# OmicsML/dance

Measured on NVIDIA H100. Metric: cells/sec fwd+bwd scGNN, higher is better.
Workload: dtype f32 (wgmma 3xTF32 split GEMMs, fp32 everything else)

## Files before the change

dance_b200/csrc/gemm_tc.cu:

```cuda
#include "tc_common.cuh"

#include <cuda_bf16.h>
#include <stdlib.h>
#include <string.h>

namespace b2 {
namespace tc {

constexpr int BM = 128;
constexpr int BK = 32;
constexpr int CONSUMERS = 256;
constexpr int REWRITERS = 128;
constexpr int THREADS = CONSUMERS + REWRITERS;
constexpr int REWRITE_REGS = 80, CONSUMER_REGS = 208;
constexpr int MAX_STAGES = 4;
constexpr int SMEM_LIMIT = 227 * 1024;

enum Mode { MODE_TF32 = 0, MODE_TF32X3 = 1, MODE_BF16 = 2 };
__host__ __device__ constexpr int plane_row_bytes(int mode) { return mode == MODE_BF16 ? BK * 2 : BK * 4; }

struct Params {
  CUtensorMap tmA;
  CUtensorMap tmB;
  float* C;
  const float* bias;
  const float* mask;
  float* partial;
  long long ldc, ldmask;
  int M, N, K;
  int a_mn, b_mn;
  int mode;
  int act;
  float beta;
  int tiles_m, tiles_n, splits, kb_per_split, kb_total, stages, planes;
};

struct SmemLayout {
  uint32_t a_plane, b_plane, plane_buf, raw_a, raw_stage, ring, bars, total;
};
__host__ __device__ inline SmemLayout smem_layout(int BN, int mode, int stages, int planes) {
  SmemLayout L;
  L.a_plane = BM * plane_row_bytes(mode);
  L.b_plane = (uint32_t)BN * plane_row_bytes(mode);
  L.plane_buf = (mode == MODE_TF32X3 ? 2u : 1u) * (L.a_plane + L.b_plane);
  L.raw_a = BM * BK * 4;
  L.raw_stage = L.raw_a + (uint32_t)BN * BK * 4;
  L.ring = (uint32_t)planes * L.plane_buf;
  L.bars = L.ring + (uint32_t)stages * L.raw_stage;
  L.total = L.bars + 8 * 4 * MAX_STAGES;
  return L;
}

template <int MODE, int ROWS, bool MN>
__device__ __forceinline__ void convert_tile(const uint8_t* raw, uint8_t* hi, uint8_t* lo, int lt) {
  constexpr int PER = ROWS * (BK / 4) / REWRITERS;
  float4 v[PER];
#pragma unroll
  for (int j = 0; j < PER; ++j) {
    const int c = lt + j * REWRITERS;
    if constexpr (!MN) {
      v[j] = *reinterpret_cast<const float4*>(raw + (c >> 3) * 128 + (c & 7) * 16);
    } else {
      const float* col = reinterpret_cast<const float*>(raw) + c % ROWS + (c / ROWS) * 4 * ROWS;
      v[j] = make_float4(col[0], col[ROWS], col[2 * ROWS], col[3 * ROWS]);
    }
  }
#pragma unroll
  for (int j = 0; j < PER; ++j) {
    const int c = lt + j * REWRITERS;
    const uint32_t r = MN ? c % ROWS : c >> 3, kc = MN ? c / ROWS : c & 7;
    if constexpr (MODE == MODE_BF16) {
      const __nv_bfloat162 p0 = __floats2bfloat162_rn(v[j].x, v[j].y), p1 = __floats2bfloat162_rn(v[j].z, v[j].w);
      *reinterpret_cast<uint2*>(hi + sw64_offset16(r, kc * 4)) =
          make_uint2(*reinterpret_cast<const uint32_t*>(&p0), *reinterpret_cast<const uint32_t*>(&p1));
      continue;
    }
    const uint32_t off = sw128_offset32(r, kc * 4);
    if constexpr (MODE == MODE_TF32X3) {
      const float4 x = v[j];
      const float4 h = make_float4(__uint_as_float(__float_as_uint(x.x) & 0xFFFFE000u), __uint_as_float(__float_as_uint(x.y) & 0xFFFFE000u),
                                   __uint_as_float(__float_as_uint(x.z) & 0xFFFFE000u), __uint_as_float(__float_as_uint(x.w) & 0xFFFFE000u));
      *reinterpret_cast<float4*>(hi + off) = h;
      *reinterpret_cast<float4*>(lo + off) = make_float4(x.x - h.x, x.y - h.y, x.z - h.z, x.w - h.w);
    } else {
      *reinterpret_cast<float4*>(hi + off) = v[j];
    }
  }
}

template <int BN>
__device__ __forceinline__ void mma_ss(float (&d)[BN / 2], uint64_t a, uint64_t b, uint32_t scale_d) {
  if constexpr (BN == 32) wgmma_tf32_ss_n32(d, a, b, scale_d);
  else if constexpr (BN == 64) wgmma_tf32_ss_n64(d, a, b, scale_d);
  else wgmma_tf32_ss_n128(d, a, b, scale_d);
}
template <int BN>
__device__ __forceinline__ void mma_bf16_ss(float (&d)[BN / 2], uint64_t a, uint64_t b, uint32_t scale_d) {
  if constexpr (BN == 32) wgmma_bf16_ss_n32(d, a, b, scale_d);
  else if constexpr (BN == 64) wgmma_bf16_ss_n64(d, a, b, scale_d);
  else wgmma_bf16_ss_n128(d, a, b, scale_d);
}

template <int BN, int MODE>
__global__ void __launch_bounds__(THREADS, 1)
gemm_tc_kernel(const __grid_constant__ Params p) {
  extern __shared__ __align__(1024) uint8_t smem_raw[];
  uint8_t* smem = smem_raw + ((1024u - (smem_u32(smem_raw) & 1023u)) & 1023u);
  const SmemLayout L = smem_layout(BN, MODE, p.stages, p.planes);
  const uint32_t raw_full = smem_u32(smem + L.bars), raw_empty = raw_full + 8 * MAX_STAGES;
  const uint32_t plane_full = raw_empty + 8 * MAX_STAGES, plane_empty = plane_full + 8 * MAX_STAGES;
  const int tid = threadIdx.x, wg = tid >> 7, lt = tid & 127;

  const int u = blockIdx.x;
  const int ks = u % p.splits;
  const int t = u / p.splits;
  const int tn = t % p.tiles_n, tm = t / p.tiles_n;
  const int kb0 = ks * p.kb_per_split;
  const int nk = min(p.kb_total, kb0 + p.kb_per_split) - kb0;
  auto plane_ptrs = [&](int b, uint8_t*& a_hi, uint8_t*& a_lo, uint8_t*& b_hi, uint8_t*& b_lo) {
    a_hi = smem + b * L.plane_buf;
    a_lo = a_hi + L.a_plane;
    b_hi = a_hi + (MODE == MODE_TF32X3 ? 2 : 1) * L.a_plane;
    b_lo = b_hi + L.b_plane;
  };

  if (tid == 0) {
    tma_prefetch_desc(&p.tmA);
    tma_prefetch_desc(&p.tmB);
    for (int s = 0; s < p.stages; ++s) {
      mbar_init(raw_full + 8 * s, 1);
      mbar_init(raw_empty + 8 * s, REWRITERS);
    }
    for (int b = 0; b < p.planes; ++b) {
      mbar_init(plane_full + 8 * b, REWRITERS);
      mbar_init(plane_empty + 8 * b, CONSUMERS / 32);
    }
    fence_barrier_init();
  }
  __syncthreads();

  if (wg == 2) {
    asm volatile("setmaxnreg.dec.sync.aligned.u32 %0;" ::"n"(REWRITE_REGS));
    auto issue = [&](int i) {
      const int s = i % p.stages, kb = kb0 + i;
      const uint32_t fb = raw_full + 8 * s;
      const uint32_t ra = smem_u32(smem + L.ring + s * L.raw_stage), rb = ra + L.raw_a;
      mbar_expect_tx(fb, L.raw_stage);
      if (!p.a_mn) tma_load_2d(ra, &p.tmA, fb, kb * BK, tm * BM);
      else tma_load_2d(ra, &p.tmA, fb, tm * BM, kb * BK);
      if (!p.b_mn) tma_load_2d(rb, &p.tmB, fb, kb * BK, tn * BN);
      else tma_load_2d(rb, &p.tmB, fb, tn * BN, kb * BK);
    };
    if (lt == 0)
      for (int i = 0; i < min(nk, p.stages); ++i) issue(i);
    for (int i = 0; i < nk; ++i) {
      if (lt == 0 && i >= 1 && i - 1 + p.stages < nk) {
        mbar_wait(raw_empty + 8 * ((i - 1) % p.stages), (uint32_t)(((i - 1) / p.stages) & 1));
        issue(i - 1 + p.stages);
      }
      const int s = i % p.stages, b = i % p.planes;
      if (i >= p.planes) mbar_wait(plane_empty + 8 * b, (uint32_t)(((i / p.planes) - 1) & 1));
      mbar_wait(raw_full + 8 * s, (uint32_t)((i / p.stages) & 1));
      uint8_t *a_hi, *a_lo, *b_hi, *b_lo;
      plane_ptrs(b, a_hi, a_lo, b_hi, b_lo);
      const uint8_t* raw = smem + L.ring + s * L.raw_stage;
      if (p.a_mn) convert_tile<MODE, BM, true>(raw, a_hi, a_lo, lt);
      else convert_tile<MODE, BM, false>(raw, a_hi, a_lo, lt);
      if (p.b_mn) convert_tile<MODE, BN, true>(raw + L.raw_a, b_hi, b_lo, lt);
      else convert_tile<MODE, BN, false>(raw + L.raw_a, b_hi, b_lo, lt);
      mbar_arrive(raw_empty + 8 * s);
      fence_proxy_async();
      mbar_arrive(plane_full + 8 * b);
    }
    return;
  }

  asm volatile("setmaxnreg.inc.sync.aligned.u32 %0;" ::"n"(CONSUMER_REGS));
  float acc[BN / 2], acc_s[BN / 2];
  const int lane = lt & 31;
  for (int i = 0; i < nk; ++i) {
    const int b = i % p.planes;
    uint8_t *a_hi, *a_lo, *b_hi, *b_lo;
    plane_ptrs(b, a_hi, a_lo, b_hi, b_lo);
    mbar_wait(plane_full + 8 * b, (uint32_t)((i / p.planes) & 1));
    wgmma_fence();
    const uint32_t ah = smem_u32(a_hi) + wg * 64 * plane_row_bytes(MODE), al = smem_u32(a_lo) + wg * 64 * plane_row_bytes(MODE);
    const uint32_t bh = smem_u32(b_hi), bl = smem_u32(b_lo);
    if constexpr (MODE == MODE_BF16) {
#pragma unroll
      for (int k = 0; k < BK / 16; ++k) {
        const uint32_t ko = k * 16 * 2;
        mma_bf16_ss<BN>(acc, wgmma_desc_sw64(ah + ko), wgmma_desc_sw64(bh + ko), (i | k) != 0);
      }
    } else {
#pragma unroll
      for (int k = 0; k < BK / 8; ++k) {
        const uint32_t ko = k * 8 * 4;
        if constexpr (MODE == MODE_TF32X3) {
          mma_ss<BN>(acc_s, wgmma_desc_sw128(al + ko), wgmma_desc_sw128(bh + ko), (i | k) != 0);
          mma_ss<BN>(acc_s, wgmma_desc_sw128(ah + ko), wgmma_desc_sw128(bl + ko), 1);
        }
        mma_ss<BN>(acc, wgmma_desc_sw128(ah + ko), wgmma_desc_sw128(bh + ko), (i | k) != 0);
      }
    }
    wgmma_commit();
    wgmma_wait<1>();
    if (i >= 1 && lane == 0) mbar_arrive(plane_empty + 8 * ((i - 1) % p.planes));
  }
  wgmma_wait<0>();
  reg_fence(acc);
  if constexpr (MODE == MODE_TF32X3) reg_fence(acc_s);

  const int warp = lt >> 5;
  const int row_base = tm * BM + wg * 64 + warp * 16 + (lane >> 2);
  const bool vec_ok = ((p.ldc & 1) == 0) && ((reinterpret_cast<uintptr_t>(p.C) & 7) == 0);
#pragma unroll
  for (int v = 0; v < BN / 2; v += 2) {
    const int row = row_base + 8 * ((v >> 1) & 1);
    const int col = tn * BN + 8 * (v >> 2) + 2 * (lane & 3);
    if (row >= p.M || col >= p.N) continue;
    float o[2] = {acc[v], acc[v + 1]};
    if constexpr (MODE == MODE_TF32X3) { o[0] += acc_s[v]; o[1] += acc_s[v + 1]; }
    const bool two = col + 1 < p.N;
    if (p.partial) {
      float* dst = p.partial + ((size_t)ks * p.M + row) * p.N + col;
      dst[0] = o[0];
      if (two) dst[1] = o[1];
      continue;
    }
    float* dst = p.C + (size_t)row * p.ldc + col;
    const float* mrow = p.mask ? p.mask + (size_t)row * p.ldmask + col : nullptr;
#pragma unroll
    for (int jj = 0; jj < 2; ++jj) {
      if (jj == 1 && !two) break;
      float x = o[jj];
      if (p.bias) x += __ldg(p.bias + col + jj);
      x = apply_act(x, p.act);
      if (mrow && !(__ldg(mrow + jj) > 0.f)) x = 0.f;
      if (p.beta != 0.f) x = fmaf(p.beta, dst[jj], x);
      o[jj] = x;
    }
    if (two && vec_ok) *reinterpret_cast<float2*>(dst) = make_float2(o[0], o[1]);
    else { dst[0] = o[0]; if (two) dst[1] = o[1]; }
  }
}

__global__ void __launch_bounds__(256)
splitk_reduce_kernel(const float* __restrict__ partial, int splits, int M, int N, float* __restrict__ C, long long ldc,
                     const float* __restrict__ bias, int act, const float* __restrict__ mask, long long ldmask,
                     float beta) {
  const size_t total = (size_t)M * N;
  for (size_t i = (size_t)blockIdx.x * blockDim.x + threadIdx.x; i < total; i += (size_t)gridDim.x * blockDim.x) {
    const int r = (int)(i / N), c = (int)(i % N);
    float s = 0.f;
    for (int k = 0; k < splits; ++k) s += partial[(size_t)k * total + i];
    if (bias) s += bias[c];
    s = apply_act(s, act);
    if (mask && !(mask[(size_t)r * ldmask + c] > 0.f)) s = 0.f;
    float* dst = C + (size_t)r * ldc + c;
    if (beta != 0.f) s = fmaf(beta, *dst, s);
    *dst = s;
  }
}

typedef CUresult (*EncodeTiledFn)(CUtensorMap*, CUtensorMapDataType, cuuint32_t, void*, const cuuint64_t*,
                                  const cuuint64_t*, const cuuint32_t*, const cuuint32_t*, CUtensorMapInterleave,
                                  CUtensorMapSwizzle, CUtensorMapL2promotion, CUtensorMapFloatOOBfill);

static EncodeTiledFn get_encode() {
  static EncodeTiledFn fn = nullptr;
  static bool tried = false;
// ... 59 lines not shown
    splits = ceil_div(sms, tiles);
    const int max_splits = pl.kb_total / 4;
    if (splits > max_splits) splits = max_splits;
    if (splits < 1) splits = 1;
  }
  pl.kb_per_split = ceil_div(pl.kb_total, splits);
  pl.splits = ceil_div(pl.kb_total, pl.kb_per_split);
  return pl;
}

template <int BN, int MODE>
static int launch_gemm(const Params& p, const Plan& pl, cudaStream_t st) {
  static bool attr_set = false;
  if (!attr_set) {
    B2_CHECK_CUDA(cudaFuncSetAttribute(gemm_tc_kernel<BN, MODE>, cudaFuncAttributeMaxDynamicSharedMemorySize, SMEM_LIMIT));
    attr_set = true;
  }
  gemm_tc_kernel<BN, MODE><<<pl.tiles_m * pl.tiles_n * pl.splits, THREADS, pl.smem, st>>>(p);
  B2_CHECK_LAUNCH("gemm_tc_kernel");
  return B2_OK;
}

template <int MODE>
static int launch_gemm_mode(const Params& p, const Plan& pl, cudaStream_t st) {
  return pl.BN == 32 ? launch_gemm<32, MODE>(p, pl, st) : (pl.BN == 64 ? launch_gemm<64, MODE>(p, pl, st) : launch_gemm<128, MODE>(p, pl, st));
}

static int mode_of(int precision) {
  return precision == B2_PREC_TF32X3 ? MODE_TF32X3 : (precision == B2_PREC_BF16 ? MODE_BF16 : MODE_TF32);
}

}

size_t gemm_tc_workspace_bytes(int M, int N, int K, int transA, int transB, int precision) {
  if (M <= 0 || N <= 0 || K <= 0) return 0;
  const tc::Plan pl = tc::make_plan(M, N, K, tc::mode_of(precision));
  return pl.splits > 1 ? (size_t)pl.splits * M * N * sizeof(float) : 0;
}

int gemm_tc(const float* A, int64_t lda, int transA, const float* B, int64_t ldb, int transB, float* C, int64_t ldc,
            int M, int N, int K, const float* bias, int act, const float* mask, int64_t ldmask, float beta,
            int precision, void* workspace, size_t workspace_bytes, cudaStream_t st) {
  using namespace tc;
  if (K < 8 || (int64_t)M * N * K < (1ll << 18)) return B2_ERR_UNSUPPORTED;
  if ((reinterpret_cast<uintptr_t>(A) & 15) || (reinterpret_cast<uintptr_t>(B) & 15) || (lda & 3) || (ldb & 3))
    return B2_ERR_UNSUPPORTED;
  if (!get_encode()) return B2_ERR_UNSUPPORTED;

  const int mode = mode_of(precision);
  const Plan pl = make_plan(M, N, K, mode);
  Params p;
  memset(&p, 0, sizeof(p));
  const int NONE = (int)CU_TENSOR_MAP_SWIZZLE_NONE;
  const bool okA = transA ? make_tensor_map_f32_ex(&p.tmA, A, (uint64_t)M, (uint64_t)K, (uint64_t)lda, BM, BK, NONE)
                          : make_tensor_map_f32_ex(&p.tmA, A, (uint64_t)K, (uint64_t)M, (uint64_t)lda, BK, BM, NONE);
  const bool okB = transB ? make_tensor_map_f32_ex(&p.tmB, B, (uint64_t)K, (uint64_t)N, (uint64_t)ldb, BK, (uint32_t)pl.BN, NONE)
                          : make_tensor_map_f32_ex(&p.tmB, B, (uint64_t)N, (uint64_t)K, (uint64_t)ldb, (uint32_t)pl.BN, BK, NONE);
  if (!okA || !okB) return B2_ERR_UNSUPPORTED;
  p.C = C; p.bias = bias; p.mask = mask; p.ldc = ldc; p.ldmask = ldmask;
  p.M = M; p.N = N; p.K = K;
  p.a_mn = transA ? 1 : 0;
  p.b_mn = transB ? 0 : 1;
  p.mode = mode; p.act = act; p.beta = beta;
  p.tiles_m = pl.tiles_m; p.tiles_n = pl.tiles_n; p.splits = pl.splits; p.kb_per_split = pl.kb_per_split;
  p.kb_total = pl.kb_total; p.stages = pl.stages; p.planes = pl.planes;
  p.partial = nullptr;
  if (pl.splits > 1) {
    const size_t need = (size_t)pl.splits * M * N * sizeof(float);
    if (!workspace || workspace_bytes < need) {
      set_error("b2_gemm_f32: split-K workspace too small (%zu < %zu)", workspace_bytes, need);
      return B2_ERR_WORKSPACE;
    }
    p.partial = reinterpret_cast<float*>(workspace);
  }
  const int rc = mode == MODE_TF32X3 ? launch_gemm_mode<MODE_TF32X3>(p, pl, st)
               : (mode == MODE_BF16 ? launch_gemm_mode<MODE_BF16>(p, pl, st) : launch_gemm_mode<MODE_TF32>(p, pl, st));
  if (rc != B2_OK) return rc;
  if (pl.splits > 1) {
    size_t total = (size_t)M * N;
    int blocks = (int)((total + 255) / 256);
    if (blocks > sm_count() * 8) blocks = sm_count() * 8;
    splitk_reduce_kernel<<<blocks, 256, 0, st>>>(p.partial, pl.splits, M, N, C, ldc, bias, act, mask, ldmask, beta);
    B2_CHECK_LAUNCH("splitk_reduce_kernel");
  }
  return B2_OK;
}

}
```

dance_b200/csrc/tc_common.cuh:

```cuda
#pragma once
#include "common.cuh"

#include <cuda.h>

namespace b2 {
namespace tc {

__device__ __forceinline__ uint32_t smem_u32(const void* p) { return (uint32_t)__cvta_generic_to_shared(p); }

__device__ __forceinline__ void mbar_init(uint32_t bar, uint32_t count) {
  asm volatile("mbarrier.init.shared::cta.b64 [%0], %1;" ::"r"(bar), "r"(count));
}
__device__ __forceinline__ void mbar_expect_tx(uint32_t bar, uint32_t bytes) {
  asm volatile("mbarrier.arrive.expect_tx.shared::cta.b64 _, [%0], %1;" ::"r"(bar), "r"(bytes) : "memory");
}
__device__ __forceinline__ void mbar_arrive(uint32_t bar) {
  asm volatile("mbarrier.arrive.shared::cta.b64 _, [%0];" ::"r"(bar) : "memory");
}
__device__ __forceinline__ void mbar_wait(uint32_t bar, uint32_t parity) {
  asm volatile(
      "{\n\t"
      ".reg .pred p;\n\t"
      "WAIT_LOOP:\n\t"
      "mbarrier.try_wait.parity.shared::cta.b64 p, [%0], %1, %2;\n\t"
// ... 8 lines not shown
               : "=r"(ok) : "r"(bar), "r"(parity) : "memory");
  return ok != 0;
}
__device__ __forceinline__ void fence_barrier_init() { asm volatile("fence.mbarrier_init.release.cluster;" ::: "memory"); }
__device__ __forceinline__ void fence_proxy_async() { asm volatile("fence.proxy.async.shared::cta;" ::: "memory"); }
__device__ __forceinline__ void tma_load_2d(uint32_t dst, const CUtensorMap* map, uint32_t bar, int c0, int c1) {
  asm volatile(
      "cp.async.bulk.tensor.2d.shared::cluster.global.mbarrier::complete_tx::bytes [%0], [%1, {%3, %4}], [%2];"
      ::"r"(dst), "l"(map), "r"(bar), "r"(c0), "r"(c1) : "memory");
}
__device__ __forceinline__ void tma_prefetch_desc(const CUtensorMap* map) {
  asm volatile("prefetch.tensormap [%0];" ::"l"(map) : "memory");
}

__device__ __forceinline__ void bulk_load(uint32_t dst, const void* src, uint32_t bytes, uint32_t bar) {
  asm volatile("cp.async.bulk.shared::cluster.global.mbarrier::complete_tx::bytes [%0], [%1], %2, [%3];"
               ::"r"(dst), "l"(src), "r"(bytes), "r"(bar) : "memory");
}

__device__ __forceinline__ uint64_t wgmma_desc_sw128(uint32_t saddr) {
  uint64_t d = 0;
  d |= (uint64_t)((saddr & 0x3FFFF) >> 4);
  d |= (uint64_t)1 << 16;
  d |= (uint64_t)(1024 >> 4) << 32;
  d |= (uint64_t)1 << 62;
  return d;
}
__host__ __device__ __forceinline__ uint32_t sw128_offset32(uint32_t row, uint32_t k) {
  return row * 128u + ((((k >> 2) ^ row) & 7u) << 4) + (k & 3u) * 4u;
}
__device__ __forceinline__ uint64_t wgmma_desc_sw64(uint32_t saddr) {
  uint64_t d = 0;
  d |= (uint64_t)((saddr & 0x3FFFF) >> 4);
  d |= (uint64_t)1 << 16;
  d |= (uint64_t)(512 >> 4) << 32;
  d |= (uint64_t)2 << 62;
  return d;
}
__host__ __device__ __forceinline__ uint32_t sw64_offset16(uint32_t row, uint32_t k) {
  return row * 64u + ((((k >> 3) ^ (row >> 1)) & 3u) << 4) + (k & 7u) * 2u;
}
__host__ __device__ __forceinline__ uint32_t sw128_offset16(uint32_t row, uint32_t k) {
  return row * 128u + ((((k >> 3) ^ row) & 7u) << 4) + (k & 7u) * 2u;
}
__device__ __forceinline__ void wgmma_fence() { asm volatile("wgmma.fence.sync.aligned;" ::: "memory"); }
__device__ __forceinline__ void wgmma_commit() { asm volatile("wgmma.commit_group.sync.aligned;" ::: "memory"); }
template <int N>
__device__ __forceinline__ void wgmma_wait() { asm volatile("wgmma.wait_group.sync.aligned %0;" ::"n"(N) : "memory"); }
template <int R>
__device__ __forceinline__ void reg_fence(float (&d)[R]) {
#pragma unroll
  for (int i = 0; i < R; ++i) asm volatile("" : "+f"(d[i])::"memory");
}

__device__ __forceinline__ void wgmma_tf32_ss_n32(float (&d)[16], uint64_t a, uint64_t b, uint32_t scale_d) {
  asm volatile(
      "{\n\t.reg .pred p;\n\tsetp.ne.b32 p, %18, 0;\n\t"
      "wgmma.mma_async.sync.aligned.m64n32k8.f32.tf32.tf32 {%0, %1, %2, %3, %4, %5, %6, %7, %8, %9, %10, %11, %12, %13, %14, %15}, %16, %17, p, 1, 1;\n\t}\n"
      : "+f"(d[0]), "+f"(d[1]), "+f"(d[2]), "+f"(d[3]), "+f"(d[4]), "+f"(d[5]), "+f"(d[6]), "+f"(d[7]), "+f"(d[8]), "+f"(d[9]), "+f"(d[10]), "+f"(d[11]), "+f"(d[12]), "+f"(d[13]), "+f"(d[14]), "+f"(d[15])
      : "l"(a), "l"(b), "r"(scale_d));
}
__device__ __forceinline__ void wgmma_tf32_ss_n64(float (&d)[32], uint64_t a, uint64_t b, uint32_t scale_d) {
  asm volatile(
      "{\n\t.reg .pred p;\n\tsetp.ne.b32 p, %34, 0;\n\t"
      "wgmma.mma_async.sync.aligned.m64n64k8.f32.tf32.tf32 {%0, %1, %2, %3, %4, %5, %6, %7, %8, %9, %10, %11, %12, %13, %14, %15, %16, %17, %18, %19, %20, %21, %22, %23, %24, %25, %26, %27, %28, %29, %30, %31}, %32, %33, p, 1, 1;\n\t}\n"
      : "+f"(d[0]), "+f"(d[1]), "+f"(d[2]), "+f"(d[3]), "+f"(d[4]), "+f"(d[5]), "+f"(d[6]), "+f"(d[7]), "+f"(d[8]), "+f"(d[9]), "+f"(d[10]), "+f"(d[11]), "+f"(d[12]), "+f"(d[13]), "+f"(d[14]), "+f"(d[15]), "+f"(d[16]), "+f"(d[17]), "+f"(d[18]), "+f"(d[19]), "+f"(d[20]), "+f"(d[21]), "+f"(d[22]), "+f"(d[23]), "+f"(d[24]), "+f"(d[25]), "+f"(d[26]), "+f"(d[27]), "+f"(d[28]), "+f"(d[29]), "+f"(d[30]), "+f"(d[31])
      : "l"(a), "l"(b), "r"(scale_d));
}
__device__ __forceinline__ void wgmma_tf32_ss_n128(float (&d)[64], uint64_t a, uint64_t b, uint32_t scale_d) {
  asm volatile(
      "{\n\t.reg .pred p;\n\tsetp.ne.b32 p, %66, 0;\n\t"
      "wgmma.mma_async.sync.aligned.m64n128k8.f32.tf32.tf32 {%0, %1, %2, %3, %4, %5, %6, %7, %8, %9, %10, %11, %12, %13, %14, %15, %16, %17, %18, %19, %20, %21, %22, %23, %24, %25, %26, %27, %28, %29, %30, %31, %32, %33, %34, %35, %36, %37, %38, %39, %40, %41, %42, %43, %44, %45, %46, %47, %48, %49, %50, %51, %52, %53, %54, %55, %56, %57, %58, %59, %60, %61, %62, %63}, %64, %65, p, 1, 1;\n\t}\n"
      : "+f"(d[0]), "+f"(d[1]), "+f"(d[2]), "+f"(d[3]), "+f"(d[4]), "+f"(d[5]), "+f"(d[6]), "+f"(d[7]), "+f"(d[8]), "+f"(d[9]), "+f"(d[10]), "+f"(d[11]), "+f"(d[12]), "+f"(d[13]), "+f"(d[14]), "+f"(d[15]), "+f"(d[16]), "+f"(d[17]), "+f"(d[18]), "+f"(d[19]), "+f"(d[20]), "+f"(d[21]), "+f"(d[22]), "+f"(d[23]), "+f"(d[24]), "+f"(d[25]), "+f"(d[26]), "+f"(d[27]), "+f"(d[28]), "+f"(d[29]), "+f"(d[30]), "+f"(d[31]), "+f"(d[32]), "+f"(d[33]), "+f"(d[34]), "+f"(d[35]), "+f"(d[36]), "+f"(d[37]), "+f"(d[38]), "+f"(d[39]), "+f"(d[40]), "+f"(d[41]), "+f"(d[42]), "+f"(d[43]), "+f"(d[44]), "+f"(d[45]), "+f"(d[46]), "+f"(d[47]), "+f"(d[48]), "+f"(d[49]), "+f"(d[50]), "+f"(d[51]), "+f"(d[52]), "+f"(d[53]), "+f"(d[54]), "+f"(d[55]), "+f"(d[56]), "+f"(d[57]), "+f"(d[58]), "+f"(d[59]), "+f"(d[60]), "+f"(d[61]), "+f"(d[62]), "+f"(d[63])
      : "l"(a), "l"(b), "r"(scale_d));
}
__device__ __forceinline__ void wgmma_f16_ss_n64(float (&d)[32], uint64_t a, uint64_t b, uint32_t scale_d) {
  asm volatile(
      "{\n\t.reg .pred p;\n\tsetp.ne.b32 p, %34, 0;\n\t"
      "wgmma.mma_async.sync.aligned.m64n64k16.f32.f16.f16 {%0, %1, %2, %3, %4, %5, %6, %7, %8, %9, %10, %11, %12, %13, %14, %15, %16, %17, %18, %19, %20, %21, %22, %23, %24, %25, %26, %27, %28, %29, %30, %31}, %32, %33, p, 1, 1, 0, 0;\n\t}\n"
      : "+f"(d[0]), "+f"(d[1]), "+f"(d[2]), "+f"(d[3]), "+f"(d[4]), "+f"(d[5]), "+f"(d[6]), "+f"(d[7]), "+f"(d[8]), "+f"(d[9]), "+f"(d[10]), "+f"(d[11]), "+f"(d[12]), "+f"(d[13]), "+f"(d[14]), "+f"(d[15]), "+f"(d[16]), "+f"(d[17]), "+f"(d[18]), "+f"(d[19]), "+f"(d[20]), "+f"(d[21]), "+f"(d[22]), "+f"(d[23]), "+f"(d[24]), "+f"(d[25]), "+f"(d[26]), "+f"(d[27]), "+f"(d[28]), "+f"(d[29]), "+f"(d[30]), "+f"(d[31])
      : "l"(a), "l"(b), "r"(scale_d));
}
__device__ __forceinline__ void wgmma_bf16_ss_n32(float (&d)[16], uint64_t a, uint64_t b, uint32_t scale_d) {
  asm volatile(
      "{\n\t.reg .pred p;\n\tsetp.ne.b32 p, %18, 0;\n\t"
      "wgmma.mma_async.sync.aligned.m64n32k16.f32.bf16.bf16 {%0, %1, %2, %3, %4, %5, %6, %7, %8, %9, %10, %11, %12, %13, %14, %15}, %16, %17, p, 1, 1, 0, 0;\n\t}\n"
      : "+f"(d[0]), "+f"(d[1]), "+f"(d[2]), "+f"(d[3]), "+f"(d[4]), "+f"(d[5]), "+f"(d[6]), "+f"(d[7]), "+f"(d[8]), "+f"(d[9]), "+f"(d[10]), "+f"(d[11]), "+f"(d[12]), "+f"(d[13]), "+f"(d[14]), "+f"(d[15])
      : "l"(a), "l"(b), "r"(scale_d));
}
__device__ __forceinline__ void wgmma_bf16_ss_n64(float (&d)[32], uint64_t a, uint64_t b, uint32_t scale_d) {
  asm volatile(
      "{\n\t.reg .pred p;\n\tsetp.ne.b32 p, %34, 0;\n\t"
      "wgmma.mma_async.sync.aligned.m64n64k16.f32.bf16.bf16 {%0, %1, %2, %3, %4, %5, %6, %7, %8, %9, %10, %11, %12, %13, %14, %15, %16, %17, %18, %19, %20, %21, %22, %23, %24, %25, %26, %27, %28, %29, %30, %31}, %32, %33, p, 1, 1, 0, 0;\n\t}\n"
      : "+f"(d[0]), "+f"(d[1]), "+f"(d[2]), "+f"(d[3]), "+f"(d[4]), "+f"(d[5]), "+f"(d[6]), "+f"(d[7]), "+f"(d[8]), "+f"(d[9]), "+f"(d[10]), "+f"(d[11]), "+f"(d[12]), "+f"(d[13]), "+f"(d[14]), "+f"(d[15]), "+f"(d[16]), "+f"(d[17]), "+f"(d[18]), "+f"(d[19]), "+f"(d[20]), "+f"(d[21]), "+f"(d[22]), "+f"(d[23]), "+f"(d[24]), "+f"(d[25]), "+f"(d[26]), "+f"(d[27]), "+f"(d[28]), "+f"(d[29]), "+f"(d[30]), "+f"(d[31])
      : "l"(a), "l"(b), "r"(scale_d));
}
__device__ __forceinline__ void wgmma_bf16_ss_n128(float (&d)[64], uint64_t a, uint64_t b, uint32_t scale_d) {
  asm volatile(
      "{\n\t.reg .pred p;\n\tsetp.ne.b32 p, %66, 0;\n\t"
      "wgmma.mma_async.sync.aligned.m64n128k16.f32.bf16.bf16 {%0, %1, %2, %3, %4, %5, %6, %7, %8, %9, %10, %11, %12, %13, %14, %15, %16, %17, %18, %19, %20, %21, %22, %23, %24, %25, %26, %27, %28, %29, %30, %31, %32, %33, %34, %35, %36, %37, %38, %39, %40, %41, %42, %43, %44, %45, %46, %47, %48, %49, %50, %51, %52, %53, %54, %55, %56, %57, %58, %59, %60, %61, %62, %63}, %64, %65, p, 1, 1, 0, 0;\n\t}\n"
      : "+f"(d[0]), "+f"(d[1]), "+f"(d[2]), "+f"(d[3]), "+f"(d[4]), "+f"(d[5]), "+f"(d[6]), "+f"(d[7]), "+f"(d[8]), "+f"(d[9]), "+f"(d[10]), "+f"(d[11]), "+f"(d[12]), "+f"(d[13]), "+f"(d[14]), "+f"(d[15]), "+f"(d[16]), "+f"(d[17]), "+f"(d[18]), "+f"(d[19]), "+f"(d[20]), "+f"(d[21]), "+f"(d[22]), "+f"(d[23]), "+f"(d[24]), "+f"(d[25]), "+f"(d[26]), "+f"(d[27]), "+f"(d[28]), "+f"(d[29]), "+f"(d[30]), "+f"(d[31]), "+f"(d[32]), "+f"(d[33]), "+f"(d[34]), "+f"(d[35]), "+f"(d[36]), "+f"(d[37]), "+f"(d[38]), "+f"(d[39]), "+f"(d[40]), "+f"(d[41]), "+f"(d[42]), "+f"(d[43]), "+f"(d[44]), "+f"(d[45]), "+f"(d[46]), "+f"(d[47]), "+f"(d[48]), "+f"(d[49]), "+f"(d[50]), "+f"(d[51]), "+f"(d[52]), "+f"(d[53]), "+f"(d[54]), "+f"(d[55]), "+f"(d[56]), "+f"(d[57]), "+f"(d[58]), "+f"(d[59]), "+f"(d[60]), "+f"(d[61]), "+f"(d[62]), "+f"(d[63])
      : "l"(a), "l"(b), "r"(scale_d));
}
__device__ __forceinline__ void wgmma_tf32_rs_n8(float (&d)[4], const uint32_t (&a)[4], uint64_t b, uint32_t scale_d) {
  asm volatile(
      "{\n\t.reg .pred p;\n\tsetp.ne.b32 p, %9, 0;\n\t"
      "wgmma.mma_async.sync.aligned.m64n8k8.f32.tf32.tf32 {%0, %1, %2, %3}, {%4, %5, %6, %7}, %8, p, 1, 1;\n\t}\n"
      : "+f"(d[0]), "+f"(d[1]), "+f"(d[2]), "+f"(d[3])
      : "r"(a[0]), "r"(a[1]), "r"(a[2]), "r"(a[3]), "l"(b), "r"(scale_d));
}
__device__ __forceinline__ void wgmma_tf32_rs_n16(float (&d)[8], const uint32_t (&a)[4], uint64_t b, uint32_t scale_d) {
  asm volatile(
      "{\n\t.reg .pred p;\n\tsetp.ne.b32 p, %13, 0;\n\t"
      "wgmma.mma_async.sync.aligned.m64n16k8.f32.tf32.tf32 {%0, %1, %2, %3, %4, %5, %6, %7}, {%8, %9, %10, %11}, %12, p, 1, 1;\n\t}\n"
      : "+f"(d[0]), "+f"(d[1]), "+f"(d[2]), "+f"(d[3]), "+f"(d[4]), "+f"(d[5]), "+f"(d[6]), "+f"(d[7])
      : "r"(a[0]), "r"(a[1]), "r"(a[2]), "r"(a[3]), "l"(b), "r"(scale_d));
}
__device__ __forceinline__ void wgmma_tf32_rs_n32(float (&d)[16], const uint32_t (&a)[4], uint64_t b, uint32_t scale_d) {
  asm volatile(
      "{\n\t.reg .pred p;\n\tsetp.ne.b32 p, %21, 0;\n\t"
      "wgmma.mma_async.sync.aligned.m64n32k8.f32.tf32.tf32 {%0, %1, %2, %3, %4, %5, %6, %7, %8, %9, %10, %11, %12, %13, %14, %15}, {%16, %17, %18, %19}, %20, p, 1, 1;\n\t}\n"
      : "+f"(d[0]), "+f"(d[1]), "+f"(d[2]), "+f"(d[3]), "+f"(d[4]), "+f"(d[5]), "+f"(d[6]), "+f"(d[7]), "+f"(d[8]), "+f"(d[9]), "+f"(d[10]), "+f"(d[11]), "+f"(d[12]), "+f"(d[13]), "+f"(d[14]), "+f"(d[15])
      : "r"(a[0]), "r"(a[1]), "r"(a[2]), "r"(a[3]), "l"(b), "r"(scale_d));
}

__device__ __forceinline__ void wgmma_f16_ss_n8(float (&d)[4], uint64_t a, uint64_t b, uint32_t scale_d) {
  asm volatile(
      "{\n\t.reg .pred p;\n\tsetp.ne.b32 p, %6, 0;\n\t"
      "wgmma.mma_async.sync.aligned.m64n8k16.f32.f16.f16 {%0, %1, %2, %3}, %4, %5, p, 1, 1, 0, 0;\n\t}\n"
      : "+f"(d[0]), "+f"(d[1]), "+f"(d[2]), "+f"(d[3])
      : "l"(a), "l"(b), "r"(scale_d));
}
__device__ __forceinline__ void wgmma_f16_ss_n16(float (&d)[8], uint64_t a, uint64_t b, uint32_t scale_d) {
  asm volatile(
      "{\n\t.reg .pred p;\n\tsetp.ne.b32 p, %10, 0;\n\t"
      "wgmma.mma_async.sync.aligned.m64n16k16.f32.f16.f16 {%0, %1, %2, %3, %4, %5, %6, %7}, %8, %9, p, 1, 1, 0, 0;\n\t}\n"
      : "+f"(d[0]), "+f"(d[1]), "+f"(d[2]), "+f"(d[3]), "+f"(d[4]), "+f"(d[5]), "+f"(d[6]), "+f"(d[7])
      : "l"(a), "l"(b), "r"(scale_d));
}
__device__ __forceinline__ void wgmma_f16_ss_n32(float (&d)[16], uint64_t a, uint64_t b, uint32_t scale_d) {
  asm volatile(
      "{\n\t.reg .pred p;\n\tsetp.ne.b32 p, %18, 0;\n\t"
      "wgmma.mma_async.sync.aligned.m64n32k16.f32.f16.f16 {%0, %1, %2, %3, %4, %5, %6, %7, %8, %9, %10, %11, %12, %13, %14, %15}, %16, %17, p, 1, 1, 0, 0;\n\t}\n"
      : "+f"(d[0]), "+f"(d[1]), "+f"(d[2]), "+f"(d[3]), "+f"(d[4]), "+f"(d[5]), "+f"(d[6]), "+f"(d[7]), "+f"(d[8]), "+f"(d[9]), "+f"(d[10]), "+f"(d[11]), "+f"(d[12]), "+f"(d[13]), "+f"(d[14]), "+f"(d[15])
      : "l"(a), "l"(b), "r"(scale_d));
}
__device__ __forceinline__ void wgmma_f16_rs_n8(float (&d)[4], const uint32_t (&a)[4], uint64_t b, uint32_t scale_d) {
  asm volatile(
      "{\n\t.reg .pred p;\n\tsetp.ne.b32 p, %9, 0;\n\t"
      "wgmma.mma_async.sync.aligned.m64n8k16.f32.f16.f16 {%0, %1, %2, %3}, {%4, %5, %6, %7}, %8, p, 1, 1, 0;\n\t}\n"
      : "+f"(d[0]), "+f"(d[1]), "+f"(d[2]), "+f"(d[3])
      : "r"(a[0]), "r"(a[1]), "r"(a[2]), "r"(a[3]), "l"(b), "r"(scale_d));
}
__device__ __forceinline__ void wgmma_f16_rs_n16(float (&d)[8], const uint32_t (&a)[4], uint64_t b, uint32_t scale_d) {
  asm volatile(
      "{\n\t.reg .pred p;\n\tsetp.ne.b32 p, %13, 0;\n\t"
      "wgmma.mma_async.sync.aligned.m64n16k16.f32.f16.f16 {%0, %1, %2, %3, %4, %5, %6, %7}, {%8, %9, %10, %11}, %12, p, 1, 1, 0;\n\t}\n"
      : "+f"(d[0]), "+f"(d[1]), "+f"(d[2]), "+f"(d[3]), "+f"(d[4]), "+f"(d[5]), "+f"(d[6]), "+f"(d[7])
      : "r"(a[0]), "r"(a[1]), "r"(a[2]), "r"(a[3]), "l"(b), "r"(scale_d));
}
__device__ __forceinline__ void wgmma_f16_rs_n32(float (&d)[16], const uint32_t (&a)[4], uint64_t b, uint32_t scale_d) {
  asm volatile(
      "{\n\t.reg .pred p;\n\tsetp.ne.b32 p, %21, 0;\n\t"
      "wgmma.mma_async.sync.aligned.m64n32k16.f32.f16.f16 {%0, %1, %2, %3, %4, %5, %6, %7, %8, %9, %10, %11, %12, %13, %14, %15}, {%16, %17, %18, %19}, %20, p, 1, 1, 0;\n\t}\n"
      : "+f"(d[0]), "+f"(d[1]), "+f"(d[2]), "+f"(d[3]), "+f"(d[4]), "+f"(d[5]), "+f"(d[6]), "+f"(d[7]), "+f"(d[8]), "+f"(d[9]), "+f"(d[10]), "+f"(d[11]), "+f"(d[12]), "+f"(d[13]), "+f"(d[14]), "+f"(d[15])
      : "r"(a[0]), "r"(a[1]), "r"(a[2]), "r"(a[3]), "l"(b), "r"(scale_d));
}
__device__ __forceinline__ void wgmma_f16_rs_n64(float (&d)[32], const uint32_t (&a)[4], uint64_t b, uint32_t scale_d) {
  asm volatile(
      "{\n\t.reg .pred p;\n\tsetp.ne.b32 p, %37, 0;\n\t"
      "wgmma.mma_async.sync.aligned.m64n64k16.f32.f16.f16 {%0, %1, %2, %3, %4, %5, %6, %7, %8, %9, %10, %11, %12, %13, %14, %15, %16, %17, %18, %19, %20, %21, %22, %23, %24, %25, %26, %27, %28, %29, %30, %31}, {%32, %33, %34, %35}, %36, p, 1, 1, 0;\n\t}\n"
      : "+f"(d[0]), "+f"(d[1]), "+f"(d[2]), "+f"(d[3]), "+f"(d[4]), "+f"(d[5]), "+f"(d[6]), "+f"(d[7]), "+f"(d[8]), "+f"(d[9]), "+f"(d[10]), "+f"(d[11]), "+f"(d[12]), "+f"(d[13]), "+f"(d[14]), "+f"(d[15]), "+f"(d[16]), "+f"(d[17]), "+f"(d[18]), "+f"(d[19]), "+f"(d[20]), "+f"(d[21]), "+f"(d[22]), "+f"(d[23]), "+f"(d[24]), "+f"(d[25]), "+f"(d[26]), "+f"(d[27]), "+f"(d[28]), "+f"(d[29]), "+f"(d[30]), "+f"(d[31])
      : "r"(a[0]), "r"(a[1]), "r"(a[2]), "r"(a[3]), "l"(b), "r"(scale_d));
}

bool make_tensor_map_f16_ex(CUtensorMap* map, const void* ptr, uint64_t inner, uint64_t outer, uint64_t ld, uint32_t box_inner,
                            uint32_t box_outer, int swizzle );
// ... 7 lines not shown
```

Baseline: 1.225 million.

## Feed A operand from registers in 3xTF32 GEMM, split hi/lo in consumers

In 3xTF32 mode the consumer warpgroups now load the A tile straight from the raw TMA stage into registers (ldmatrix or swizzled pair loads) and split it into hi/lo themselves. They then issue register-sourced wgmma, so the A hi/lo smem planes and the rewriter's A conversion go away. The A tensor map switches to 128B swizzle and is loaded in 32-row boxes for the transposed case. Register budgets are rebalanced toward consumers, and B conversion is batched to fit the smaller rewriter budget. This shortens the rewriter critical path and frees shared memory, at the cost of more consumer register pressure and a new cross-role barrier dependency on the raw stage.

```diff
diff --git a/dance_b200/csrc/gemm_tc.cu b/dance_b200/csrc/gemm_tc.cu
--- a/dance_b200/csrc/gemm_tc.cu
+++ b/dance_b200/csrc/gemm_tc.cu
@@ -12,12 +12,14 @@
 constexpr int CONSUMERS = 256;
 constexpr int REWRITERS = 128;
 constexpr int THREADS = CONSUMERS + REWRITERS;
-constexpr int REWRITE_REGS = 80, CONSUMER_REGS = 208;
+enum Mode { MODE_TF32 = 0, MODE_TF32X3 = 1, MODE_BF16 = 2 };
+__host__ __device__ constexpr int rewrite_regs(int mode) { return mode == MODE_TF32X3 ? 56 : 80; }
+__host__ __device__ constexpr int consumer_regs(int mode) { return mode == MODE_TF32X3 ? 224 : 208; }
 constexpr int MAX_STAGES = 4;
 constexpr int SMEM_LIMIT = 227 * 1024;
 
-enum Mode { MODE_TF32 = 0, MODE_TF32X3 = 1, MODE_BF16 = 2 };
 __host__ __device__ constexpr int plane_row_bytes(int mode) { return mode == MODE_BF16 ? BK * 2 : BK * 4; }
+constexpr int MN_BOX_ROWS = 32, MN_BOX_BYTES = MN_BOX_ROWS * BK * 4;
 
 struct Params {
   CUtensorMap tmA;
@@ -40,7 +42,7 @@
 };
 __host__ __device__ inline SmemLayout smem_layout(int BN, int mode, int stages, int planes) {
   SmemLayout L;
-  L.a_plane = BM * plane_row_bytes(mode);
+  L.a_plane = mode == MODE_TF32X3 ? 0u : BM * plane_row_bytes(mode);
   L.b_plane = (uint32_t)BN * plane_row_bytes(mode);
   L.plane_buf = (mode == MODE_TF32X3 ? 2u : 1u) * (L.a_plane + L.b_plane);
   L.raw_a = BM * BK * 4;
@@ -51,39 +53,43 @@
   return L;
 }
 
-template <int MODE, int ROWS, bool MN>
+template <int MODE, int ROWS, bool MN, int BATCH = ROWS * (BK / 4) / REWRITERS>
 __device__ __forceinline__ void convert_tile(const uint8_t* raw, uint8_t* hi, uint8_t* lo, int lt) {
   constexpr int PER = ROWS * (BK / 4) / REWRITERS;
-  float4 v[PER];
-#pragma unroll
-  for (int j = 0; j < PER; ++j) {
-    const int c = lt + j * REWRITERS;
-    if constexpr (!MN) {
-      v[j] = *reinterpret_cast<const float4*>(raw + (c >> 3) * 128 + (c & 7) * 16);
-    } else {
-      const float* col = reinterpret_cast<const float*>(raw) + c % ROWS + (c / ROWS) * 4 * ROWS;
-      v[j] = make_float4(col[0], col[ROWS], col[2 * ROWS], col[3 * ROWS]);
-    }
-  }
-#pragma unroll
-  for (int j = 0; j < PER; ++j) {
-    const int c = lt + j * REWRITERS;
-    const uint32_t r = MN ? c % ROWS : c >> 3, kc = MN ? c / ROWS : c & 7;
-    if constexpr (MODE == MODE_BF16) {
-      const __nv_bfloat162 p0 = __floats2bfloat162_rn(v[j].x, v[j].y), p1 = __floats2bfloat162_rn(v[j].z, v[j].w);
-      *reinterpret_cast<uint2*>(hi + sw64_offset16(r, kc * 4)) =
-          make_uint2(*reinterpret_cast<const uint32_t*>(&p0), *reinterpret_cast<const uint32_t*>(&p1));
-      continue;
-    }
-    const uint32_t off = sw128_offset32(r, kc * 4);
-    if constexpr (MODE == MODE_TF32X3) {
-      const float4 x = v[j];
-      const float4 h = make_float4(__uint_as_float(__float_as_uint(x.x) & 0xFFFFE000u), __uint_as_float(__float_as_uint(x.y) & 0xFFFFE000u),
-                                   __uint_as_float(__float_as_uint(x.z) & 0xFFFFE000u), __uint_as_float(__float_as_uint(x.w) & 0xFFFFE000u));
-      *reinterpret_cast<float4*>(hi + off) = h;
-      *reinterpret_cast<float4*>(lo + off) = make_float4(x.x - h.x, x.y - h.y, x.z - h.z, x.w - h.w);
-    } else {
-      *reinterpret_cast<float4*>(hi + off) = v[j];
+  static_assert(PER % BATCH == 0, "whole batches");
+#pragma unroll
+  for (int j0 = 0; j0 < PER; j0 += BATCH) {
+    float4 v[BATCH];
+#pragma unroll
+    for (int j = 0; j < BATCH; ++j) {
+      const int c = lt + (j0 + j) * REWRITERS;
+      if constexpr (!MN) {
+        v[j] = *reinterpret_cast<const float4*>(raw + (c >> 3) * 128 + (c & 7) * 16);
+      } else {
+        const float* col = reinterpret_cast<const float*>(raw) + c % ROWS + (c / ROWS) * 4 * ROWS;
+        v[j] = make_float4(col[0], col[ROWS], col[2 * ROWS], col[3 * ROWS]);
+      }
+    }
+#pragma unroll
+    for (int j = 0; j < BATCH; ++j) {
+      const int c = lt + (j0 + j) * REWRITERS;
+      const uint32_t r = MN ? c % ROWS : c >> 3, kc = MN ? c / ROWS : c & 7;
+      if constexpr (MODE == MODE_BF16) {
+        const __nv_bfloat162 p0 = __floats2bfloat162_rn(v[j].x, v[j].y), p1 = __floats2bfloat162_rn(v[j].z, v[j].w);
+        *reinterpret_cast<uint2*>(hi + sw64_offset16(r, kc * 4)) =
+            make_uint2(*reinterpret_cast<const uint32_t*>(&p0), *reinterpret_cast<const uint32_t*>(&p1));
+        continue;
+      }
+      const uint32_t off = sw128_offset32(r, kc * 4);
+      if constexpr (MODE == MODE_TF32X3) {
+        const float4 x = v[j];
+        const float4 h = make_float4(__uint_as_float(__float_as_uint(x.x) & 0xFFFFE000u), __uint_as_float(__float_as_uint(x.y) & 0xFFFFE000u),
+                                     __uint_as_float(__float_as_uint(x.z) & 0xFFFFE000u), __uint_as_float(__float_as_uint(x.w) & 0xFFFFE000u));
+        *reinterpret_cast<float4*>(hi + off) = h;
+        *reinterpret_cast<float4*>(lo + off) = make_float4(x.x - h.x, x.y - h.y, x.z - h.z, x.w - h.w);
+      } else {
+        *reinterpret_cast<float4*>(hi + off) = v[j];
+      }
     }
   }
 }
@@ -95,10 +101,21 @@
   else wgmma_tf32_ss_n128(d, a, b, scale_d);
 }
 template <int BN>
+__device__ __forceinline__ void mma_rs(float (&d)[BN / 2], const uint32_t (&a)[4], uint64_t b, uint32_t scale_d) {
+  if constexpr (BN == 32) wgmma_tf32_rs_n32(d, a, b, scale_d);
+  else if constexpr (BN == 64) wgmma_tf32_rs_n64(d, a, b, scale_d);
+  else wgmma_tf32_rs_n128(d, a, b, scale_d);
+}
+template <int BN>
 __device__ __forceinline__ void mma_bf16_ss(float (&d)[BN / 2], uint64_t a, uint64_t b, uint32_t scale_d) {
   if constexpr (BN == 32) wgmma_bf16_ss_n32(d, a, b, scale_d);
   else if constexpr (BN == 64) wgmma_bf16_ss_n64(d, a, b, scale_d);
   else wgmma_bf16_ss_n128(d, a, b, scale_d);
+}
+
+__device__ __forceinline__ int mn_pair_row(int warp, int lane) {
+  const int g = lane >> 2;
+  return MN_BOX_ROWS * (warp >> 1) + 4 * (2 * (warp & 1) + (g >> 2) + 4 * ((g >> 1) & 1)) + 2 * (g & 1);
 }
 
 template <int BN, int MODE>
@@ -129,7 +146,7 @@
     tma_prefetch_desc(&p.tmB);
     for (int s = 0; s < p.stages; ++s) {
       mbar_init(raw_full + 8 * s, 1);
-      mbar_init(raw_empty + 8 * s, REWRITERS);
+      mbar_init(raw_empty + 8 * s, REWRITERS + (MODE == MODE_TF32X3 ? CONSUMERS / 32 : 0));
     }
     for (int b = 0; b < p.planes; ++b) {
       mbar_init(plane_full + 8 * b, REWRITERS);
@@ -140,13 +157,16 @@
   __syncthreads();
 
   if (wg == 2) {
-    asm volatile("setmaxnreg.dec.sync.aligned.u32 %0;" ::"n"(REWRITE_REGS));
+    asm volatile("setmaxnreg.dec.sync.aligned.u32 %0;" ::"n"(rewrite_regs(MODE)));
+    const int a_boxes = MODE == MODE_TF32X3 && p.a_mn ? min(BM / MN_BOX_ROWS, (p.M - tm * BM + MN_BOX_ROWS - 1) / MN_BOX_ROWS) : 0;
     auto issue = [&](int i) {
       const int s = i % p.stages, kb = kb0 + i;
       const uint32_t fb = raw_full + 8 * s;
       const uint32_t ra = smem_u32(smem + L.ring + s * L.raw_stage), rb = ra + L.raw_a;
-      mbar_expect_tx(fb, L.raw_stage);
-      if (!p.a_mn) tma_load_2d(ra, &p.tmA, fb, kb * BK, tm * BM);
+      mbar_expect_tx(fb, L.raw_stage - (a_boxes ? (BM / MN_BOX_ROWS - a_boxes) * MN_BOX_BYTES : 0));
+      if (a_boxes)
+        for (int j = 0; j < a_boxes; ++j) tma_load_2d(ra + j * MN_BOX_BYTES, &p.tmA, fb, tm * BM + j * MN_BOX_ROWS, kb * BK);
+      else if (!p.a_mn) tma_load_2d(ra, &p.tmA, fb, kb * BK, tm * BM);
       else tma_load_2d(ra, &p.tmA, fb, tm * BM, kb * BK);
       if (!p.b_mn) tma_load_2d(rb, &p.tmB, fb, kb * BK, tn * BN);
       else tma_load_2d(rb, &p.tmB, fb, tn * BN, kb * BK);
@@ -164,10 +184,13 @@
       uint8_t *a_hi, *a_lo, *b_hi, *b_lo;
       plane_ptrs(b, a_hi, a_lo, b_hi, b_lo);
       const uint8_t* raw = smem + L.ring + s * L.raw_stage;
-      if (p.a_mn) convert_tile<MODE, BM, true>(raw, a_hi, a_lo, lt);
-      else convert_tile<MODE, BM, false>(raw, a_hi, a_lo, lt);
-      if (p.b_mn) convert_tile<MODE, BN, true>(raw + L.raw_a, b_hi, b_lo, lt);
-      else convert_tile<MODE, BN, false>(raw + L.raw_a, b_hi, b_lo, lt);
+      if constexpr (MODE != MODE_TF32X3) {
+        if (p.a_mn) convert_tile<MODE, BM, true>(raw, a_hi, a_lo, lt);
+        else convert_tile<MODE, BM, false>(raw, a_hi, a_lo, lt);
+      }
+      constexpr int B_BATCH = MODE == MODE_TF32X3 && BN == 128 ? 4 : BN * (BK / 4) / REWRITERS;
+      if (p.b_mn) convert_tile<MODE, BN, true, B_BATCH>(raw + L.raw_a, b_hi, b_lo, lt);
+      else convert_tile<MODE, BN, false, B_BATCH>(raw + L.raw_a, b_hi, b_lo, lt);
       mbar_arrive(raw_empty + 8 * s);
       fence_proxy_async();
       mbar_arrive(plane_full + 8 * b);
@@ -175,48 +198,109 @@
     return;
   }
 
-  asm volatile("setmaxnreg.inc.sync.aligned.u32 %0;" ::"n"(CONSUMER_REGS));
+  asm volatile("setmaxnreg.inc.sync.aligned.u32 %0;" ::"n"(consumer_regs(MODE)));
   float acc[BN / 2], acc_s[BN / 2];
-  const int lane = lt & 31;
-  for (int i = 0; i < nk; ++i) {
-    const int b = i % p.planes;
-    uint8_t *a_hi, *a_lo, *b_hi, *b_lo;
-    plane_ptrs(b, a_hi, a_lo, b_hi, b_lo);
-    mbar_wait(plane_full + 8 * b, (uint32_t)((i / p.planes) & 1));
-    wgmma_fence();
-    const uint32_t ah = smem_u32(a_hi) + wg * 64 * plane_row_bytes(MODE), al = smem_u32(a_lo) + wg * 64 * plane_row_bytes(MODE);
-    const uint32_t bh = smem_u32(b_hi), bl = smem_u32(b_lo);
-    if constexpr (MODE == MODE_BF16) {
-#pragma unroll
-      for (int k = 0; k < BK / 16; ++k) {
-        const uint32_t ko = k * 16 * 2;
-        mma_bf16_ss<BN>(acc, wgmma_desc_sw64(ah + ko), wgmma_desc_sw64(bh + ko), (i | k) != 0);
-      }
+  const int warp = lt >> 5, lane = lt & 31;
+  int row0 = tm * BM + wg * 64 + warp * 16 + (lane >> 2), row_step = 8;
+  if constexpr (MODE == MODE_TF32X3) {
+    uint32_t a_off[BK / 8];
+    if (p.a_mn) {
+      const int m = wg * 64 + mn_pair_row(warp, lane), t = lane & 3, c = (m & (MN_BOX_ROWS - 1)) >> 2;
+      const uint32_t box = (m / MN_BOX_ROWS) * MN_BOX_BYTES + (m & 3) * 4;
+      a_off[0] = box + t * 128 + ((c ^ t) << 4);
+      a_off[1] = box + (t + 4) * 128 + ((c ^ (t + 4)) << 4);
+      row0 = tm * BM + m;
+      row_step = 1;
     } else {
+      const int r = wg * 64 + warp * 16 + (lane & 7) + 8 * ((lane >> 3) & 1);
+#pragma unroll
+      for (int kk = 0; kk < BK / 8; ++kk) a_off[kk] = r * 128 + ((((2 * kk) | (lane >> 4)) ^ (lane & 7)) << 4);
+    }
+    auto kblock = [&](int i, uint32_t (&hi)[BK / 8][4], uint32_t (&lo)[BK / 8][4]) {
+      const int s = i % p.stages, b = i % p.planes;
+      const uint8_t* raw = smem + L.ring + s * L.raw_stage;
+      mbar_wait(raw_full + 8 * s, (uint32_t)((i / p.stages) & 1));
+      if (p.a_mn) {
+#pragma unroll
+        for (int kk = 0; kk < BK / 8; ++kk) {
+          const uint2 x0 = *reinterpret_cast<const uint2*>(raw + kk * 1024 + a_off[0]);
+          const uint2 x1 = *reinterpret_cast<const uint2*>(raw + kk * 1024 + a_off[1]);
+          hi[kk][0] = x0.x; hi[kk][1] = x0.y; hi[kk][2] = x1.x; hi[kk][3] = x1.y;
+        }
+      } else {
+#pragma unroll
+        for (int kk = 0; kk < BK / 8; ++kk) ldsm_x4(hi[kk], smem_u32(raw) + a_off[kk]);
+      }
+#pragma unroll
+      for (int kk = 0; kk < BK / 8; ++kk)
+#pragma unroll
+        for (int j = 0; j < 4; ++j) {
+          const uint32_t x = hi[kk][j];
+          hi[kk][j] = x & 0xFFFFE000u;
+          lo[kk][j] = __float_as_uint(__uint_as_float(x) - __uint_as_float(hi[kk][j]));
+        }
+#pragma unroll
+      for (int kk = 0; kk < BK / 8; ++kk) {
+        reg_fence(hi[kk]);
+        reg_fence(lo[kk]);
+      }
+      __syncwarp();
+      if (lane == 0) mbar_arrive(raw_empty + 8 * s);
+      mbar_wait(plane_full + 8 * b, (uint32_t)((i / p.planes) & 1));
+      wgmma_fence();
+      const uint32_t bh = smem_u32(smem + b * L.plane_buf), bl = bh + L.b_plane;
 #pragma unroll
       for (int k = 0; k < BK / 8; ++k) {
         const uint32_t ko = k * 8 * 4;
-        if constexpr (MODE == MODE_TF32X3) {
-          mma_ss<BN>(acc_s, wgmma_desc_sw128(al + ko), wgmma_desc_sw128(bh + ko), (i | k) != 0);
-          mma_ss<BN>(acc_s, wgmma_desc_sw128(ah + ko), wgmma_desc_sw128(bl + ko), 1);
+        mma_rs<BN>(acc_s, lo[k], wgmma_desc_sw128(bh + ko), (i | k) != 0);
+        mma_rs<BN>(acc_s, hi[k], wgmma_desc_sw128(bl + ko), 1);
+        mma_rs<BN>(acc, hi[k], wgmma_desc_sw128(bh + ko), (i | k) != 0);
+      }
+      wgmma_commit();
+      wgmma_wait<1>();
+      if (i >= 1 && lane == 0) mbar_arrive(plane_empty + 8 * ((i - 1) % p.planes));
+    };
+    uint32_t hi0[BK / 8][4], lo0[BK / 8][4], hi1[BK / 8][4], lo1[BK / 8][4];
+    int i = 0;
+    for (; i + 1 < nk; i += 2) {
+      kblock(i, hi0, lo0);
+      kblock(i + 1, hi1, lo1);
+    }
+    if (i < nk) kblock(i, hi0, lo0);
+  } else {
+    for (int i = 0; i < nk; ++i) {
+      const int b = i % p.planes;
+      uint8_t *a_hi, *a_lo, *b_hi, *b_lo;
+      plane_ptrs(b, a_hi, a_lo, b_hi, b_lo);
+      mbar_wait(plane_full + 8 * b, (uint32_t)((i / p.planes) & 1));
+      wgmma_fence();
+      const uint32_t ah = smem_u32(a_hi) + wg * 64 * plane_row_bytes(MODE), bh = smem_u32(b_hi);
+      if constexpr (MODE == MODE_BF16) {
+#pragma unroll
+        for (int k = 0; k < BK / 16; ++k) {
+          const uint32_t ko = k * 16 * 2;
+          mma_bf16_ss<BN>(acc, wgmma_desc_sw64(ah + ko), wgmma_desc_sw64(bh + ko), (i | k) != 0);
         }
-        mma_ss<BN>(acc, wgmma_desc_sw128(ah + ko), wgmma_desc_sw128(bh + ko), (i | k) != 0);
-      }
-    }
-    wgmma_commit();
-    wgmma_wait<1>();
-    if (i >= 1 && lane == 0) mbar_arrive(plane_empty + 8 * ((i - 1) % p.planes));
+      } else {
+#pragma unroll
+        for (int k = 0; k < BK / 8; ++k) {
+          const uint32_t ko = k * 8 * 4;
+          mma_ss<BN>(acc, wgmma_desc_sw128(ah + ko), wgmma_desc_sw128(bh + ko), (i | k) != 0);
+        }
+      }
+      wgmma_commit();
+      wgmma_wait<1>();
+      if (i >= 1 && lane == 0) mbar_arrive(plane_empty + 8 * ((i - 1) % p.planes));
+    }
   }
   wgmma_wait<0>();
   reg_fence(acc);
   if constexpr (MODE == MODE_TF32X3) reg_fence(acc_s);
 
-  const int warp = lt >> 5;
-  const int row_base = tm * BM + wg * 64 + warp * 16 + (lane >> 2);
   const bool vec_ok = ((p.ldc & 1) == 0) && ((reinterpret_cast<uintptr_t>(p.C) & 7) == 0);
 #pragma unroll
   for (int v = 0; v < BN / 2; v += 2) {
-    const int row = row_base + 8 * ((v >> 1) & 1);
+    const int row = row0 + row_step * ((v >> 1) & 1);
     const int col = tn * BN + 8 * (v >> 2) + 2 * (lane & 3);
     if (row >= p.M || col >= p.N) continue;
     float o[2] = {acc[v], acc[v + 1]};
@@ -382,8 +466,10 @@
   Params p;
   memset(&p, 0, sizeof(p));
   const int NONE = (int)CU_TENSOR_MAP_SWIZZLE_NONE;
-  const bool okA = transA ? make_tensor_map_f32_ex(&p.tmA, A, (uint64_t)M, (uint64_t)K, (uint64_t)lda, BM, BK, NONE)
-                          : make_tensor_map_f32_ex(&p.tmA, A, (uint64_t)K, (uint64_t)M, (uint64_t)lda, BK, BM, NONE);
+  const int a_swizzle = mode == MODE_TF32X3 ? (int)CU_TENSOR_MAP_SWIZZLE_128B : NONE;
+  const bool okA = transA ? make_tensor_map_f32_ex(&p.tmA, A, (uint64_t)M, (uint64_t)K, (uint64_t)lda,
+                                                   mode == MODE_TF32X3 ? MN_BOX_ROWS : BM, BK, a_swizzle)
+                          : make_tensor_map_f32_ex(&p.tmA, A, (uint64_t)K, (uint64_t)M, (uint64_t)lda, BK, BM, a_swizzle);
   const bool okB = transB ? make_tensor_map_f32_ex(&p.tmB, B, (uint64_t)K, (uint64_t)N, (uint64_t)ldb, BK, (uint32_t)pl.BN, NONE)
                           : make_tensor_map_f32_ex(&p.tmB, B, (uint64_t)N, (uint64_t)K, (uint64_t)ldb, (uint32_t)pl.BN, BK, NONE);
   if (!okA || !okB) return B2_ERR_UNSUPPORTED;
diff --git a/dance_b200/csrc/tc_common.cuh b/dance_b200/csrc/tc_common.cuh
--- a/dance_b200/csrc/tc_common.cuh
+++ b/dance_b200/csrc/tc_common.cuh
@@ -84,6 +84,11 @@
 #pragma unroll
   for (int i = 0; i < R; ++i) asm volatile("" : "+f"(d[i])::"memory");
 }
+template <int R>
+__device__ __forceinline__ void reg_fence(uint32_t (&a)[R]) {
+#pragma unroll
+  for (int i = 0; i < R; ++i) asm volatile("" : "+r"(a[i])::"memory");
+}
 
 __device__ __forceinline__ void wgmma_tf32_ss_n32(float (&d)[16], uint64_t a, uint64_t b, uint32_t scale_d) {
   asm volatile(
@@ -155,6 +160,24 @@
       : "+f"(d[0]), "+f"(d[1]), "+f"(d[2]), "+f"(d[3]), "+f"(d[4]), "+f"(d[5]), "+f"(d[6]), "+f"(d[7]), "+f"(d[8]), "+f"(d[9]), "+f"(d[10]), "+f"(d[11]), "+f"(d[12]), "+f"(d[13]), "+f"(d[14]), "+f"(d[15])
       : "r"(a[0]), "r"(a[1]), "r"(a[2]), "r"(a[3]), "l"(b), "r"(scale_d));
 }
+__device__ __forceinline__ void wgmma_tf32_rs_n64(float (&d)[32], const uint32_t (&a)[4], uint64_t b, uint32_t scale_d) {
+  asm volatile(
+      "{\n\t.reg .pred p;\n\tsetp.ne.b32 p, %37, 0;\n\t"
+      "wgmma.mma_async.sync.aligned.m64n64k8.f32.tf32.tf32 {%0, %1, %2, %3, %4, %5, %6, %7, %8, %9, %10, %11, %12, %13, %14, %15, %16, %17, %18, %19, %20, %21, %22, %23, %24, %25, %26, %27, %28, %29, %30, %31}, {%32, %33, %34, %35}, %36, p, 1, 1;\n\t}\n"
+      : "+f"(d[0]), "+f"(d[1]), "+f"(d[2]), "+f"(d[3]), "+f"(d[4]), "+f"(d[5]), "+f"(d[6]), "+f"(d[7]), "+f"(d[8]), "+f"(d[9]), "+f"(d[10]), "+f"(d[11]), "+f"(d[12]), "+f"(d[13]), "+f"(d[14]), "+f"(d[15]), "+f"(d[16]), "+f"(d[17]), "+f"(d[18]), "+f"(d[19]), "+f"(d[20]), "+f"(d[21]), "+f"(d[22]), "+f"(d[23]), "+f"(d[24]), "+f"(d[25]), "+f"(d[26]), "+f"(d[27]), "+f"(d[28]), "+f"(d[29]), "+f"(d[30]), "+f"(d[31])
+      : "r"(a[0]), "r"(a[1]), "r"(a[2]), "r"(a[3]), "l"(b), "r"(scale_d));
+}
+__device__ __forceinline__ void wgmma_tf32_rs_n128(float (&d)[64], const uint32_t (&a)[4], uint64_t b, uint32_t scale_d) {
+  asm volatile(
+      "{\n\t.reg .pred p;\n\tsetp.ne.b32 p, %69, 0;\n\t"
+      "wgmma.mma_async.sync.aligned.m64n128k8.f32.tf32.tf32 {%0, %1, %2, %3, %4, %5, %6, %7, %8, %9, %10, %11, %12, %13, %14, %15, %16, %17, %18, %19, %20, %21, %22, %23, %24, %25, %26, %27, %28, %29, %30, %31, %32, %33, %34, %35, %36, %37, %38, %39, %40, %41, %42, %43, %44, %45, %46, %47, %48, %49, %50, %51, %52, %53, %54, %55, %56, %57, %58, %59, %60, %61, %62, %63}, {%64, %65, %66, %67}, %68, p, 1, 1;\n\t}\n"
+      : "+f"(d[0]), "+f"(d[1]), "+f"(d[2]), "+f"(d[3]), "+f"(d[4]), "+f"(d[5]), "+f"(d[6]), "+f"(d[7]), "+f"(d[8]), "+f"(d[9]), "+f"(d[10]), "+f"(d[11]), "+f"(d[12]), "+f"(d[13]), "+f"(d[14]), "+f"(d[15]), "+f"(d[16]), "+f"(d[17]), "+f"(d[18]), "+f"(d[19]), "+f"(d[20]), "+f"(d[21]), "+f"(d[22]), "+f"(d[23]), "+f"(d[24]), "+f"(d[25]), "+f"(d[26]), "+f"(d[27]), "+f"(d[28]), "+f"(d[29]), "+f"(d[30]), "+f"(d[31]), "+f"(d[32]), "+f"(d[33]), "+f"(d[34]), "+f"(d[35]), "+f"(d[36]), "+f"(d[37]), "+f"(d[38]), "+f"(d[39]), "+f"(d[40]), "+f"(d[41]), "+f"(d[42]), "+f"(d[43]), "+f"(d[44]), "+f"(d[45]), "+f"(d[46]), "+f"(d[47]), "+f"(d[48]), "+f"(d[49]), "+f"(d[50]), "+f"(d[51]), "+f"(d[52]), "+f"(d[53]), "+f"(d[54]), "+f"(d[55]), "+f"(d[56]), "+f"(d[57]), "+f"(d[58]), "+f"(d[59]), "+f"(d[60]), "+f"(d[61]), "+f"(d[62]), "+f"(d[63])
+      : "r"(a[0]), "r"(a[1]), "r"(a[2]), "r"(a[3]), "l"(b), "r"(scale_d));
+}
+__device__ __forceinline__ void ldsm_x4(uint32_t (&r)[4], uint32_t saddr) {
+  asm volatile("ldmatrix.sync.aligned.m8n8.x4.shared.b16 {%0, %1, %2, %3}, [%4];"
+               : "=r"(r[0]), "=r"(r[1]), "=r"(r[2]), "=r"(r[3]) : "r"(saddr) : "memory");
+}
 
 __device__ __forceinline__ void wgmma_f16_ss_n8(float (&d)[4], uint64_t a, uint64_t b, uint32_t scale_d) {
   asm volatile(
```

After: 1.256 million (median of 6 runs). 2.5% higher.
